# adaptivegenome/openge

Measured on AMD Instinct MI355X. Metric: Mreads/sec sort+dedup (and realign intervals/sec), 1/2/4/8 MI355X, higher is better.
Workload: dtype u8

## Files before the change

openge_amd/csrc/bgzf.hip:

```cpp
#include <hip/hip_runtime.h>

#include <cstdint>
#include <cstdlib>
#include <cstring>
#include <string>
#include <vector>

#include "bam_layout.h"
#include "oge_ctx.h"
#include "records.h"
#include "bgzf_dev.h"

namespace {

using namespace oge_bgzf;
constexpr int kT = 512;
constexpr int kSeg = 64;
constexpr int kSub = kT * kSeg;
constexpr int kNSub = 2;
constexpr int kNSeg = kT * kNSub;
constexpr int kHashBits = 12;
constexpr int kLit = 286, kDist = 30, kCl = 19;
constexpr int kFreq = kLit + kDist;
constexpr int kHdrWords = 144;
// ... 732 lines not shown
    __syncthreads();
    {
        const uint32_t c = lane >= 1 && lane <= M ? hs.cnt[lane] : 0u;
        uint32_t K = c << ((M - lane) & 31);
#pragma unroll
        for (int o = 32; o >= 1; o >>= 1) K += __shfl_xor(K, o, 64);
        if (lane == 0 && K != (1u << M)) {
            const uint32_t one = 1u << M;
            while (K > one) {
                int b = M - 1;
                while (hs.cnt[b] == 0) --b;
                hs.cnt[b]--;
                hs.cnt[b + 1]++;
                K -= 1u << (M - b - 1);
            }
            while (K < one) {
                int b = M;
                while (hs.cnt[b] == 0 || K + (1u << (M - b)) > one) --b;
                hs.cnt[b]--;
                hs.cnt[b - 1]++;
                K += 1u << (M - b);
            }
        }
    }
    __syncthreads();
    {
        uint32_t suf = lane >= 1 && lane <= M ? hs.cnt[lane] : 0u;
#pragma unroll
        for (int o = 1; o < 16; o <<= 1) {
            const uint32_t y = __shfl_down(suf, o, 64);
            if (lane + o < 16) suf += y;
        }
        uint32_t sb[15];
#pragma unroll
        for (int b = 0; b < 15; ++b) sb[b] = (uint32_t)__shfl((int)suf, b + 1, 64);
        for (uint32_t k = lane; k < m; k += 64) {
            uint32_t b = 0;
#pragma unroll
            for (int q = 0; q < 15; ++q) b += (q < M && k < sb[q]) ? 1u : 0u;
            len[hs.sorted[k]] = (uint8_t)b;
        }
    }
    __syncthreads();
    HLCLK(5);
#if OGE_EXP == 3
    if (n == kLit && blockIdx.x == 0 && threadIdx.x == 0)
        printf("huff_lengths lit: keys %llu sort %llu merge %llu depths %llu counts+lengths %llu (m %u)\n",
               (unsigned long long)(g_hl_clk[1] - g_hl_clk[0]), (unsigned long long)(g_hl_clk[2] - g_hl_clk[1]),
               (unsigned long long)(g_hl_clk[3] - g_hl_clk[2]), (unsigned long long)(g_hl_clk[4] - g_hl_clk[3]),
               (unsigned long long)(g_hl_clk[5] - g_hl_clk[4]), m);
#endif
}

__device__ void huff_codes(const uint8_t *len, int n, uint32_t *out) {
    const int lane = threadIdx.x;
    const uint64_t lt = (1ull << lane) - 1;
    uint32_t cnt = 0;
    for (int i0 = 0; i0 < n; i0 += 64) {
        const uint32_t L = i0 + lane < n ? len[i0 + lane] : 0u;
#pragma unroll
        for (int b = 1; b < 16; ++b) {
            const uint32_t c = (uint32_t)__popcll(__ballot(L == (uint32_t)b));
            if (lane == b) cnt += c;
        }
    }
    uint32_t first = 0, code = 0;
#pragma unroll
    for (int b = 1; b < 16; ++b) {
        code = (code + (b > 1 ? (uint32_t)__shfl(cnt, b - 1, 64) : 0u)) << 1;
        if (lane == b) first = code;
    }
    uint32_t run = 0;
    for (int i0 = 0; i0 < n; i0 += 64) {
        const int i = i0 + lane;
        const uint32_t L = i < n ? len[i] : 0u;
        const uint32_t base = (uint32_t)__shfl(run, (int)L, 64) + (uint32_t)__shfl(first, (int)L, 64);
        uint32_t r = 0, add = 0;
#pragma unroll
        for (int b = 1; b < 16; ++b) {
            const uint64_t mk = __ballot(L == (uint32_t)b);
            if (L == (uint32_t)b) r = (uint32_t)__popcll(mk & lt);
            if (lane == b) add = (uint32_t)__popcll(mk);
        }
        run += add;
        if (i < n) out[i] = L ? (__builtin_bitreverse32(base + r) >> (32 - L)) | (L << 16) : 0u;
    }
    __syncthreads();
}

__constant__ uint8_t kClOrder[kCl] = {16, 17, 18, 0, 8, 7, 9, 6, 10, 5, 11, 4, 12, 3, 13, 2, 14, 1, 15};

__device__ __forceinline__ uint32_t len_extra(uint32_t ls) { return ls < 8 ? 0u : ls < 28 ? (ls - 4) >> 2 : 0u; }
__device__ __forceinline__ uint32_t dist_extra(uint32_t ds) { return ds < 4 ? 0u : (ds - 2) >> 1; }

__global__ void __launch_bounds__(64) k_defl_huff(const uint32_t *__restrict__ freq_in, DeflTab *__restrict__ tabs, uint64_t n,
                                                 uint64_t blk0, int level, uint32_t *__restrict__ sizes) {
    __shared__ uint32_t f[kFreq];
    __shared__ uint8_t lens[kFreq];
    __shared__ uint32_t fcl[kCl];
    __shared__ uint8_t lcl[kCl];
    __shared__ uint32_t ccl[kCl];
    __shared__ uint8_t cl_sym[kFreq], cl_ext[kFreq];
    __shared__ uint32_t ncl;
    __shared__ HuffScratch hs;
    const int lane = threadIdx.x;
    DeflTab &T = tabs[blockIdx.x];
#if OGE_EXP == 3
    uint64_t xc[10];
    int xn = 0;
#define XCLK() (xc[xn++] = __builtin_readcyclecounter())
#else
#define XCLK()
#endif
    XCLK();
    uint32_t nzl = 0, nzd = 0;
    for (int i = lane, r = 0; r < (kFreq + 63) / 64; i += 64, ++r) {
        const uint32_t v = i < kFreq ? freq_in[(uint64_t)blockIdx.x * kFreq + i] + (i == 256) : 0u;
        if (i < kFreq) f[i] = v;
        nzl += (uint32_t)__popcll(__ballot(i < kLit && v != 0));
        nzd += (uint32_t)__popcll(__ballot(i >= kLit && i < kFreq && v != 0));
    }
    __syncthreads();
    if (lane == 0 && (nzl < 2 || nzd < 2)) {
        for (int i = 0; nzl < 2 && i < kLit; ++i)
            if (!f[i]) f[i] = 1, ++nzl;
        for (int i = 0; nzd < 2 && i < kDist; ++i)
            if (!f[kLit + i]) f[kLit + i] = 1, ++nzd;
    }
    __syncthreads();
    XCLK();
    huff_lengths(f, kLit, 15, lens, hs);
    XCLK();
    huff_lengths(f + kLit, kDist, 15, lens + kLit, hs);
    XCLK();
    huff_codes(lens, kLit, T.lit);
    huff_codes(lens + kLit, kDist, T.dist);
    XCLK();

    __shared__ uint32_t hlit, hdist;
    __shared__ uint32_t hw[kHdrWords];
    {
        uint32_t la = 0, lb = 0;
        for (int r = 0; r < 5; ++r) {
            const int i = 64 * r + lane;
            const uint64_t mk = __ballot(i < kLit && lens[i] != 0);
            if (mk) la = 64 * r + 64 - __builtin_clzll(mk);
        }
        const uint64_t mkd = __ballot(lane < kDist && lens[kLit + lane] != 0);
        if (mkd) lb = 64 - __builtin_clzll(mkd);
        const uint32_t a = max(la, 257u), b = max(lb, 1u), N = a + b;
        auto val = [&](uint32_t p) -> uint32_t { return p < a ? lens[p] : lens[kLit + p - a]; };
        uint64_t st[5];
#pragma unroll
        for (int r = 0; r < 5; ++r) {
            const uint32_t p = 64 * r + lane;
            st[r] = __ballot(p < N && (p == 0 || p == a || val(p) != val(p - 1)));
        }
        if (lane < kCl) fcl[lane] = 0;
        if (lane == 0) hlit = a, hdist = b;
        __syncthreads();
        uint32_t base = 0;
#pragma unroll
        for (int r = 0; r < 5; ++r) {
            const uint32_t p = 64 * r + lane;
            const bool start = (st[r] >> lane) & 1;
            uint32_t R = 0, v = 0, ntok = 0;
            if (start) {
                uint32_t nx = N;
                const uint64_t rest = lane < 63 ? st[r] & (~0ull << (lane + 1)) : 0ull;
                if (rest) {
                    nx = 64 * r + __builtin_ctzll(rest);
                } else {
#pragma unroll
                    for (int r2 = 4; r2 > r; --r2)
                        if (st[r2]) nx = 64 * r2 + __builtin_ctzll(st[r2]);
                }
                R = min(nx, N) - p;
                v = val(p);
                if (v == 0) {
                    const uint32_t rm = R % 138;
                    ntok = R / 138 + (rm >= 3 ? 1 : rm);
                } else {
                    const uint32_t rm = (R - 1) % 6;
                    ntok = 1 + (R - 1) / 6 + (rm >= 3 ? 1 : rm);
                }
            }
            uint32_t inc = ntok;
#pragma unroll
            for (int o = 1; o < 64; o <<= 1) {
                const uint32_t y = __shfl_up(inc, o, 64);
                if (lane >= (uint32_t)o) inc += y;
            }
            uint32_t k = base + inc - ntok;
            base += __shfl(inc, 63, 64);
            if (start) {
                auto tok = [&](uint32_t sym, uint32_t ext) {
                    cl_sym[k] = (uint8_t)sym;
                    cl_ext[k] = (uint8_t)ext;
                    atomicAdd(&fcl[sym], 1u);
                    ++k;
                };
                if (v == 0) {
                    for (uint32_t q = 0; q < R / 138; ++q) tok(18, 127);
                    const uint32_t rm = R % 138;
                    if (rm >= 11) tok(18, rm - 11);
                    else if (rm >= 3) tok(17, rm - 3);
                    else
                        for (uint32_t q = 0; q < rm; ++q) tok(0, 0);
                } else {
                    tok(v, 0);
                    for (uint32_t q = 0; q < (R - 1) / 6; ++q) tok(16, 3);
                    const uint32_t rm = (R - 1) % 6;
                    if (rm >= 3) tok(16, rm - 3);
                    else
                        for (uint32_t q = 0; q < rm; ++q) tok(v, 0);
                }
            }
        }
        __syncthreads();
        if (lane == 0) {
            ncl = base;
            uint32_t nz = 0;
            for (int i = 0; i < kCl; ++i) nz += fcl[i] != 0;
            for (int i = 0; nz < 2 && i < kCl; ++i)
                if (!fcl[i]) fcl[i] = 1, ++nz;
        }
    }
    __syncthreads();
    XCLK();
    huff_lengths(fcl, kCl, 7, lcl, hs);
    huff_codes(lcl, kCl, ccl);
    XCLK();
    {
        for (int i = lane; i < kHdrWords; i += 64) hw[i] = 0;
        const uint64_t mh = __ballot(lane >= 4 && lane < kCl && lcl[kClOrder[lane]] != 0);
        const uint32_t hclen = mh ? 64 - __builtin_clzll(mh) : 4u;
        __syncthreads();
        auto orbits = [&](uint32_t at, uint32_t v, uint32_t nb) {
            if (!nb) return;
            const uint32_t w = at >> 5, sh = at & 31;
            atomicOr(&hw[w], v << sh);
            if (sh + nb > 32) atomicOr(&hw[w + 1], v >> (32 - sh));
        };
        if (lane == 0) orbits(0, 1u | (2u << 1) | ((hlit - 257) << 3) | ((hdist - 1) << 8) | ((hclen - 4) << 13), 17);
        if ((uint32_t)lane < hclen) orbits(17 + 3 * lane, lcl[kClOrder[lane]], 3);
        const uint32_t n = ncl;
        uint32_t at = 17 + 3 * hclen;
        for (uint32_t t0 = 0; t0 < n; t0 += 64) {
            const uint32_t t = t0 + lane;
            uint32_t nb = 0, v = 0;
            if (t < n) {
                const uint32_t sym = cl_sym[t], c = ccl[sym], cb = c >> 16;
                const uint32_t eb = sym == 16 ? 2u : sym == 17 ? 3u : sym == 18 ? 7u : 0u;
                nb = cb + eb;
                v = (c & 0xffff) | ((uint32_t)cl_ext[t] << cb);
            }
            uint32_t inc = nb;
#pragma unroll
            for (int o = 1; o < 64; o <<= 1) {
                const uint32_t y = __shfl_up(inc, o, 64);
                if (lane >= (uint32_t)o) inc += y;
            }
            orbits(at + inc - nb, v, nb);
            at += __shfl(inc, 63, 64);
        }
        __syncthreads();
        for (uint32_t i = lane; i < (at + 31) / 32; i += 64) T.hdr[i] = hw[i];
        if (lane == 0) {
            T.hdr_bits = at;
            ncl = at;
        }
    }
    __syncthreads();
    uint32_t bits = 0;
    for (int i = lane; i < kFreq; i += 64) {
        const uint32_t fr = freq_in[(uint64_t)blockIdx.x * kFreq + i] + (i == 256);
        const uint32_t ex = i < 257 ? 0u : i < kLit ? len_extra(i - 257) : dist_extra(i - kLit);
        bits += fr * (lens[i] + ex);
    }
#pragma unroll
    for (int o = 32; o >= 1; o >>= 1) bits += __shfl_xor(bits, o, 64);
    if (lane == 0) {
        const uint64_t start = (blk0 + blockIdx.x) * kPay;
        const uint32_t len = (uint32_t)min<uint64_t>(kPay, n - start);
        const uint32_t dbytes = (ncl + bits + 7) / 8;
        const uint32_t stored = level == 0 || dbytes > len + 5;
        const uint32_t total = stored ? 18 + 5 + len + 8 : 18 + dbytes + 8;
        T.stored = stored;
        T.total = total;
        sizes[blockIdx.x] = total;
    }
#if OGE_EXP == 3
    XCLK();
    if (lane == 0 && blockIdx.x < 4 && blk0 == 0)
        printf("huff-exp blk %u: load %llu lit-lengths %llu dist-lengths %llu codes %llu rle %llu cl %llu header+size %llu\n",
               blockIdx.x, (unsigned long long)(xc[1] - xc[0]), (unsigned long long)(xc[2] - xc[1]), (unsigned long long)(xc[3] - xc[2]),
               (unsigned long long)(xc[4] - xc[3]), (unsigned long long)(xc[5] - xc[4]), (unsigned long long)(xc[6] - xc[5]),
               (unsigned long long)(xc[7] - xc[6]));
#endif
}

struct LdsBits {
    uint32_t *base;
    uint64_t acc;
    uint32_t nacc, wpos;
    __device__ __forceinline__ void init(uint32_t *b, uint32_t bit) { base = b, acc = 0, nacc = bit & 31, wpos = bit >> 5; }
    __device__ __forceinline__ void put(uint32_t v, uint32_t nb) {
        acc |= (uint64_t)v << nacc;
        nacc += nb;
        if (nacc >= 32) {
            const uint32_t w = (uint32_t)acc;
            atomicOr(base + wpos, w);
            ++wpos;
            acc >>= 32;
            nacc -= 32;
        }
    }
    __device__ __forceinline__ void finish() {
        if (nacc && (uint32_t)acc) atomicOr(base + wpos, (uint32_t)acc);
    }
};

__device__ __forceinline__ uint32_t ct_entry(uint32_t i, const uint32_t *tlit) {
    if (i < 256) {
        const uint32_t c = tlit[i];
        return (c & 0xffff) | (c >> 16) << 24;
    }
    uint32_t sym, nb, ev;
    len_code(i - 256 + 3, sym, nb, ev);
    const uint32_t c = tlit[sym];
    return ((c & 0xffff) | (ev << (c >> 16))) | ((c >> 16) + nb) << 24;
}
__device__ __forceinline__ void dist_bits(uint32_t D, const uint32_t *dist, uint32_t &v, uint32_t &n) {
    const uint32_t d = D - 1, lg = 31 - __builtin_clz(d | 1);
    const bool small = d < 4;
    const uint32_t dnb = small ? 0u : lg - 1;
    const uint32_t dsym = small ? d : 2 * lg + ((d >> ((lg - 1) & 31)) & 1);
    const uint32_t dev = d & ((1u << dnb) - 1);
    const uint32_t c = dist[dsym];
    v = (c & 0xffff) | (dev << (c >> 16));
    n = (c >> 16) + dnb;
}
__device__ __forceinline__ uint32_t match_bits(uint32_t m, const uint32_t *ct, const uint32_t *dist) {
    uint32_t dv, dn;
    dist_bits((m & 0x7fff) + 1, dist, dv, dn);
    return (ct[256 + ((m >> 15) & 255)] >> 24) + dn;
}

__device__ __forceinline__ void seg_load(const uint8_t *s, uint32_t s0, uint32_t len, uint32_t (&w)[16]) {
    if (s0 + kSeg <= len && !((uintptr_t)(s + s0) & 15)) {
        const uint4 *g = (const uint4 *)(s + s0);
#pragma unroll
        for (int k = 0; k < 4; ++k) {
            const uint4 v = g[k];
            w[4 * k] = v.x, w[4 * k + 1] = v.y, w[4 * k + 2] = v.z, w[4 * k + 3] = v.w;
        }
    } else {
#pragma unroll
        for (int k = 0; k < 16; ++k) {
            uint32_t v = 0;
#pragma unroll
            for (int b = 0; b < 4; ++b)
                if (s0 + 4 * k + b < len) v |= (uint32_t)s[s0 + 4 * k + b] << (8 * b);
            w[k] = v;
        }
    }
}

#ifndef OGE_EMIT_MPRE
#define OGE_EMIT_MPRE 8
#endif
constexpr int kMPre = OGE_EMIT_MPRE;
__device__ __forceinline__ void seg_tokens(const uint32_t *mp, uint32_t nm, uint32_t (&m)[kMPre]) {
    const uint32_t last = nm ? nm - 1 : 0;
#pragma unroll
    for (int k = 0; k < kMPre; ++k) m[k] = mp[(uint64_t)min((uint32_t)k, last) * kNSeg];
}

__device__ __forceinline__ uint32_t seg_bits(const uint32_t (&w)[16], uint64_t lm, uint32_t nm, const uint32_t *mp,
                                             const uint32_t (&m)[kMPre], const uint32_t *ct, const uint32_t *dist) {
    uint32_t bits = 0;
#pragma unroll
    for (int g = 0; g < 4; ++g) {
        uint32_t c[16];
#pragma unroll
        for (int i = 0; i < 16; ++i) c[i] = ct[(w[4 * g + (i >> 2)] >> (8 * (i & 3))) & 0xff];
#pragma unroll
        for (int i = 0; i < 16; ++i) bits += (lm >> (16 * g + i)) & 1 ? c[i] >> 24 : 0u;
    }
#pragma unroll
    for (int k = 0; k < kMPre; ++k)
        if ((uint32_t)k < nm) bits += match_bits(m[k], ct, dist);
    for (uint32_t k = kMPre; k < nm; ++k) bits += match_bits(mp[(uint64_t)k * kNSeg], ct, dist);
    return bits;
}

__device__ __forceinline__ void seg_emit(const uint32_t (&w)[16], uint64_t lm, uint32_t nm, const uint32_t *mp,
                                         uint32_t (&m)[kMPre], const uint32_t *ct, const uint32_t *dist, uint32_t *img,
                                         uint32_t bit) {
    uint32_t k = 0, cur = m[0], moff = nm ? (cur >> 23) : 64u;
    uint32_t lc, dv, dn;
    auto look = [&](uint32_t tok) {
        lc = ct[256 + ((tok >> 15) & 255)];
        dist_bits((tok & 0x7fff) + 1, dist, dv, dn);
    };
    look(cur);
    LdsBits bw;
    bw.init(img, bit);
#pragma unroll
    for (int g = 0; g < 4; ++g) {
        uint32_t c[16];
#pragma unroll
        for (int i = 0; i < 16; ++i) c[i] = ct[(w[4 * g + (i >> 2)] >> (8 * (i & 3))) & 0xff];
#pragma unroll
        for (int i0 = 0; i0 < 16; i0 += 2) {
            const int i = 16 * g + i0;
            const uint32_t a = (lm >> i) & 1 ? c[i0] : 0u, b = (lm >> (i + 1)) & 1 ? c[i0 + 1] : 0u;
            bw.put((a & 0xffffff) | ((b & 0xffffff) << (a >> 24)), (a >> 24) + (b >> 24));
            if (((uint32_t)i | 1u) == (moff | 1u)) {
#if OGE_EXP == 8
                ++k;
#pragma unroll
                for (int q = 0; q + 1 < kMPre; ++q) m[q] = m[q + 1];
                moff = k < nm && k < (uint32_t)kMPre ? m[0] >> 23 : 64u;
#else
                bw.put(lc & 0xffffff, lc >> 24);
                bw.put(dv, dn);
                ++k;
#pragma unroll
                for (int q = 0; q + 1 < kMPre; ++q) m[q] = m[q + 1];
                if (k < nm) {
                    cur = k < (uint32_t)kMPre ? m[0] : mp[(uint64_t)k * kNSeg];
                    moff = cur >> 23;
                    look(cur);
                } else {
                    moff = 64;
                }
#endif
            }
        }
    }
    bw.finish();
}

struct EmitCrc {
    uint32_t crctab[4][256];
    uint32_t zp[17][32];
    uint32_t zl[32][16];
    uint32_t crcs[kT / 64];
};
constexpr uint32_t kLdsGranule = 1280;
constexpr uint32_t kLdsCu = 163840;
constexpr uint32_t kEmitFixed = (512 + kDist + kNSeg + kT / 64 + 2) * 4;
constexpr uint32_t emit_lds(uint32_t cap) { return (cap + 16 + kEmitFixed + kLdsGranule - 1) / kLdsGranule * kLdsGranule; }
#ifndef OGE_EMIT_SMALL_CAP
#define OGE_EMIT_SMALL_CAP (46 * 1024)
#endif
constexpr uint32_t kEmitSmallCap = OGE_EMIT_SMALL_CAP;
static_assert(kEmitSmallCap % 1024 == 0 && 3 * emit_lds(kEmitSmallCap) <= kLdsCu && 3 * emit_lds(kEmitSmallCap + 1024) > kLdsCu,
              "small emit instance: three workgroups per CU, and no larger cap does");
static_assert(sizeof(EmitCrc) <= kEmitSmallCap, "the CRC tables alias the image");

template <uint32_t CAP>
__device__ __forceinline__ void emit_block(const uint32_t bi, const uint8_t *__restrict__ src, uint64_t n, uint64_t blk0,
                                           const uint64_t *__restrict__ lmask, const uint8_t *__restrict__ nmatch,
                                           const uint32_t *__restrict__ mlist, const DeflTab *__restrict__ tabs,
                                           const uint32_t *__restrict__ zpow, const uint32_t *__restrict__ offs,
                                           const uint64_t *__restrict__ cbase, uint8_t *__restrict__ dst) {
    constexpr bool kSmall = CAP < kSlot;
    const DeflTab &T = tabs[bi];
    const uint32_t total = T.total, stored = T.stored, hb = T.hdr_bits;
    __shared__ __align__(16) uint32_t img[CAP / 4 + 4];
    __shared__ uint32_t ct[512], dist[kDist];
    __shared__ uint32_t scan[kNSeg];
    __shared__ uint32_t wsum[kT / 64];
    __shared__ __align__(16) uint32_t crc_own[kSmall ? 1 : sizeof(EmitCrc) / 4];
    __shared__ uint32_t sh_crc;
    EmitCrc &C = *(EmitCrc *)(kSmall ? img : crc_own);
    int tid = threadIdx.x;
    asm volatile("" : "+v"(tid));
    const int t = tid, lane = t & 63, wv = t >> 6;
    const uint64_t blk = blk0 + bi;
    const uint64_t start = blk * kPay;
    const uint32_t len = (uint32_t)min<uint64_t>(kPay, n - start);
    const uint8_t *s = src + start;
    for (int i = t; i < 512; i += kT) ct[i] = ct_entry(i, T.lit);
    for (int i = t; i < kDist; i += kT) dist[i] = T.dist[i];
    crc_setup<kT>(C.crctab, C.zp, zpow, t);
    for (int i = t; i < 32 * 16; i += kT) C.zl[i >> 4][i & 15] = zpow[17 * 32 + i];
    if (!kSmall)
        for (uint32_t i = t; i < (total + 15) / 16; i += kT) ((uint4 *)img)[i] = make_uint4(0, 0, 0, 0);
    __syncthreads();
    {
        const uint32_t c = crc_global512x4l(s, len, C.crctab, C.zl, C.zp, C.crcs, t);
        if (t == 0) sh_crc = c;
    }
    if (kSmall) {
        __syncthreads();
        for (uint32_t i = t; i < (total + 15) / 16; i += kT) ((uint4 *)img)[i] = make_uint4(0, 0, 0, 0);
        if (stored) __syncthreads();
    }
    const uint32_t bsize = total - 1;
    if (stored) {
        for (uint32_t i = t; i < len; i += kT) ((uint8_t *)img)[23 + i] = s[i];
    } else {
        const uint32_t s0a = t * kSeg, s0b = kSub + t * kSeg;
        const uint64_t sga = (uint64_t)bi * kNSeg + t, sgb = sga + kT;
        const uint64_t lma = s0a < len ? lmask[sga] : 0, lmb = s0b < len ? lmask[sgb] : 0;
        const uint32_t nma = s0a < len ? nmatch[sga] : 0, nmb = s0b < len ? nmatch[sgb] : 0;
        const uint32_t *mpa = mlist + ((uint64_t)bi * kMaxM) * kNSeg + t, *mpb = mpa + kT;
        uint32_t ca, cb;
        {
            uint32_t w[16], m[kMPre];
            seg_load(s, s0a, len, w);
            seg_tokens(mpa, nma, m);
            ca = seg_bits(w, lma, nma, mpa, m, ct, dist);
            seg_load(s, s0b, len, w);
            seg_tokens(mpb, nmb, m);
            cb = seg_bits(w, lmb, nmb, mpb, m, ct, dist);
        }
        scan[t] = ca;
        scan[kT + t] = cb;
        __syncthreads();
        {
            const uint32_t a = scan[2 * t], b = scan[2 * t + 1];
            uint32_t x = a + b, inc = x;
#pragma unroll
            for (int o = 1; o < 64; o <<= 1) {
                const uint32_t y = __shfl_up(inc, o);
                if (lane >= o) inc += y;
            }
            if (lane == 63) wsum[wv] = inc;
            __syncthreads();
            uint32_t pre = 0;
            for (int q = 0; q < wv; ++q) pre += wsum[q];
            const uint32_t ex = pre + inc - x;
            __syncthreads();
            scan[2 * t] = ex;
            scan[2 * t + 1] = ex + a;
        }
        __syncthreads();
        for (uint32_t i = t; i < (hb + 31) / 32; i += kT) {
            const uint32_t v = T.hdr[i];
            atomicOr(img + 4 + i, v << 16);
            if (v >> 16) atomicOr(img + 5 + i, v >> 16);
        }
        {
            uint32_t w[16], m[kMPre];
            if (ca) {
                seg_load(s, s0a, len, w);
                seg_tokens(mpa, nma, m);
                seg_emit(w, lma, nma, mpa, m, ct, dist, img, 144 + hb + scan[t]);
            }
            if (cb) {
                uint32_t tb = t;
                asm volatile("" : "+v"(tb));
                const uint64_t lm2 = lmask[(uint64_t)bi * kNSeg + kT + tb];
                seg_load(s, s0b, len, w);
                seg_tokens(mpb, nmb, m);
                seg_emit(w, lm2, nmb, mpb, m, ct, dist, img, 144 + hb + scan[kT + t]);
            }
        }
        if (t == kT - 1) {
            const uint32_t body_end = 144 + hb + scan[kNSeg - 1] + cb;
            LdsBits bw;
            bw.init(img, body_end);
            const uint32_t c = T.lit[256];
            bw.put(c & 0xffff, c >> 16);
            bw.finish();
        }
    }
    __syncthreads();
    uint8_t *ib = (uint8_t *)img;
    if (t == 0) {
        img[0] = 0x04088b1fu;
        img[1] = 0;
        img[2] = 0x0006ff00u;
        img[3] = 0x00024342u;
        ib[16] = (uint8_t)bsize, ib[17] = (uint8_t)(bsize >> 8);
        if (stored) {
            ib[18] = 1;
            ib[19] = (uint8_t)len, ib[20] = (uint8_t)(len >> 8);
            ib[21] = (uint8_t)~len, ib[22] = (uint8_t)(~len >> 8);
        }
        const uint32_t q = total - 8;
        for (int b = 0; b < 4; ++b) ib[q + b] = (uint8_t)(sh_crc >> (8 * b)), ib[q + 4 + b] = (uint8_t)(len >> (8 * b));
    }
    __syncthreads();
    uint8_t *D = dst + *cbase + offs[bi];
    const uint32_t sh = (uint32_t)((uintptr_t)D & 3);
    OGE_G uint32_t *A = (OGE_G uint32_t *)((uintptr_t)D & ~(uintptr_t)3);
    const uint32_t nwords = (total + sh + 3) / 4;
    for (uint32_t g = t; g < nwords; g += kT) {
        const int32_t r0 = (int32_t)(4 * g) - (int32_t)sh;
        if (r0 >= 0 && r0 + 4 <= (int32_t)total) {
            A[g] = ld32(img, (uint32_t)r0);
        } else {
            for (int i = 0; i < 4; ++i) {
                const int32_t r = r0 + i;
                if (r >= 0 && r < (int32_t)total) ((OGE_G uint8_t *)(A + g))[i] = ib[r];
            }
        }
    }
}

template <uint32_t CAP>
__global__ void __launch_bounds__(kT, CAP < kSlot ? 6 : 4) k_defl_emit(const uint8_t *__restrict__ src, uint64_t n, uint64_t blk0,
                                                     const uint64_t *__restrict__ lmask, const uint8_t *__restrict__ nmatch,
                                                     const uint32_t *__restrict__ mlist, const DeflTab *__restrict__ tabs,
                                                     const uint32_t *__restrict__ zpow, const uint32_t *__restrict__ offs,
                                                     const uint64_t *__restrict__ cbase, uint8_t *__restrict__ dst, uint32_t cap,
                                                     const uint32_t *__restrict__ big) {
    if (CAP < kSlot) {
        if (tabs[blockIdx.x].total <= cap) emit_block<CAP>(blockIdx.x, src, n, blk0, lmask, nmatch, mlist, tabs, zpow, offs, cbase, dst);
    } else {
        const uint32_t nq = big ? big[0] : blockIdx.x + 1;
#pragma unroll 1
        for (uint32_t q = blockIdx.x; q < nq; q += gridDim.x) {
            const uint32_t bi = big ? big[4 + q] : q;
            if (!big && tabs[bi].total <= cap) break;
            emit_block<CAP>(bi, src, n, blk0, lmask, nmatch, mlist, tabs, zpow, offs, cbase, dst);
            __syncthreads();
        }
    }
}

constexpr uint32_t kMaxChunk = 16384, kPer = kMaxChunk / 1024;
__global__ void __launch_bounds__(1024) k_scan_chunk(const uint32_t *__restrict__ in, uint32_t n, uint32_t *__restrict__ out,
                                                     uint32_t cap, unsigned long long *__restrict__ nsmall,
                                                     uint32_t *__restrict__ big) {
    __shared__ uint32_t ws[16], wb[16];
    const uint32_t t = threadIdx.x, lane = t & 63, w = t >> 6;
    uint32_t a[kPer], v = 0, nbig = 0, small = 0;
#pragma unroll
    for (uint32_t i = 0; i < kPer; ++i) {
        a[i] = kPer * t + i < n ? in[kPer * t + i] : 0;
        v += a[i];
        small += a[i] && a[i] <= cap;
        nbig += a[i] > cap;
    }
#pragma unroll
    for (int d = 32; d >= 1; d >>= 1) small += __shfl_xor(small, d, 64);
    if (lane == 0 && small) atomicAdd(nsmall, (unsigned long long)small);
    uint32_t x = v, xb = nbig;
#pragma unroll
    for (int d = 1; d < 64; d <<= 1) {
        const uint32_t y = __shfl_up(x, d, 64), yb = __shfl_up(xb, d, 64);
        if (lane >= (uint32_t)d) x += y, xb += yb;
    }
    if (lane == 63) ws[w] = x, wb[w] = xb;
    __syncthreads();
    if (t < 16) {
        uint32_t s = ws[t], z = s, sb = wb[t], zb = sb;
        for (int d = 1; d < 16; d <<= 1) {
            const uint32_t y = __shfl_up(z, d, 16), yb = __shfl_up(zb, d, 16);
            if ((t & 15) >= (uint32_t)d) z += y, zb += yb;
        }
        ws[t] = z - s;
        wb[t] = zb - sb;
        if (t == 15) big[0] = zb;
    }
    __syncthreads();
    uint32_t excl = ws[w] + x - v, rank = wb[w] + xb - nbig;
#pragma unroll
    for (uint32_t i = 0; i < kPer; ++i) {
        if (kPer * t + i < n) out[kPer * t + i] = excl;
        excl += a[i];
        if (a[i] > cap) big[4 + rank++] = kPer * t + i;
    }
}

__global__ void k_defl_advance(uint64_t *base, uint64_t *cbase, const uint32_t *offs, const uint32_t *sizes, uint32_t nb) {
    if (threadIdx.x == 0 && blockIdx.x == 0) {
        const uint64_t b = *base;
        *cbase = b;
        *base = b + (uint64_t)offs[nb - 1] + sizes[nb - 1];
    }
}

__global__ void k_fix_bins(uint8_t *__restrict__ recs, const uint64_t *__restrict__ off, uint64_t n) {
    const uint64_t i = (uint64_t)blockIdx.x * blockDim.x + threadIdx.x;
    if (i >= n) return;
    uint8_t *r = recs + off[i];
    oge_wr_u16(r + OGE_OFF_BIN, oge_rec_bin(r));
}

}


extern "C" uint64_t oge_bgzf_bound(uint64_t n) { return ((n + kPay - 1) / kPay) * (uint64_t)kSlot; }

extern "C" uint32_t oge_defl_emit_cap(void) { return kEmitSmallCap; }

static uint32_t emit_cap_now() {
    const char *e = getenv("OGE_DEFL_EMIT_CAP");
    if (!e || !*e) return kEmitSmallCap;
    return (uint32_t)std::min<unsigned long long>(strtoull(e, nullptr, 10), kEmitSmallCap);
}

extern "C" int oge_bgzf_deflate_dev(oge_ctx *ctx, const uint8_t *d_src, uint64_t n, int level, uint8_t *d_dst,
                                    uint64_t dst_cap, uint64_t *out_bytes) {
    if (!ctx) return oge_fail(nullptr, OGE_ERR_ARG, "null ctx");
    if (!out_bytes || (n && (!d_src || !d_dst))) return oge_fail(ctx, OGE_ERR_ARG, "null buffer");
    if (level < 0 || level > 9) return oge_fail(ctx, OGE_ERR_ARG, "level must be 0..9");
    const int depth = level >= 9 ? 32 : level == 8 ? 8 : 1, lazy = level >= 8 ? 1 : 0;
    const int search = level == 0 ? OGE_DEFL_FAST : ctx->deflate_search;
    if (dst_cap < oge_bgzf_bound(n)) return oge_fail(ctx, OGE_ERR_ARG, "dst_cap < oge_bgzf_bound(n)");
    OgeCall call(ctx, false);
    *out_bytes = 0;
    if (!n) return OGE_OK;
    const uint64_t nblk = (n + kPay - 1) / kPay;
    const int ncu = ctx->cu_count();
#ifndef OGE_DEFL_STREAMS
#define OGE_DEFL_STREAMS 3
#endif
#ifndef OGE_DEFL_CHUNK
#define OGE_DEFL_CHUNK kMaxChunk
#endif
    static_assert(OGE_DEFL_CHUNK <= kMaxChunk, "k_scan_chunk bound");
    constexpr uint64_t kPerPay = (uint64_t)kNSeg * 8 + kNSeg + (uint64_t)kMaxM * kNSeg * 4 + kFreq * 4 + sizeof(DeflTab) + 8;
    const int S0 = nblk > 4096 ? OGE_DEFL_STREAMS : 1;
    uint64_t chunk = std::min<uint64_t>(nblk, OGE_DEFL_CHUNK);
    if (chunk > 4096) {
        size_t fr = 0, tot = 0;
        if (hipMemGetInfo(&fr, &tot) != hipSuccess) fr = 0;
        uint64_t held = 0;
        for (int s = 0; s < 3; ++s) {
            const auto it = ctx->bufs.find("defl_mlist" + std::to_string(s));
            if (it != ctx->bufs.end()) held += it->second.cap / ((uint64_t)kMaxM * kNSeg * 4) * kPerPay;
        }
        while (chunk > 4096 && (uint64_t)S0 * chunk * kPerPay > (fr + held) / 4) chunk = std::max<uint64_t>(4096, chunk / 2);
    }
    static_assert(OGE_DEFL_STREAMS >= 1 && OGE_DEFL_STREAMS <= 3, "deflate: 1-3 streams");
    const int S = nblk > chunk ? OGE_DEFL_STREAMS : 1;
    struct Bufs {
        uint64_t *lmask, *cbase;
        uint32_t *mlist, *freq, *sizes, *offs, *big;
        uint8_t *nmatch;
        DeflTab *tabs;
        hipStream_t st;
    } B[3];
    for (int s = 0; s < S; ++s) {
        const std::string x = std::to_string(s);
        B[s].lmask = (uint64_t *)ctx->ws(("defl_lmask" + x).c_str(), chunk * kNSeg * 8);
        B[s].nmatch = (uint8_t *)ctx->ws(("defl_nmatch" + x).c_str(), chunk * kNSeg);
        B[s].mlist = (uint32_t *)ctx->ws(("defl_mlist" + x).c_str(), chunk * kMaxM * kNSeg * 4);
        B[s].freq = (uint32_t *)ctx->ws(("defl_freq" + x).c_str(), chunk * kFreq * 4);
        B[s].tabs = (DeflTab *)ctx->ws(("defl_tabs" + x).c_str(), chunk * sizeof(DeflTab));
        B[s].sizes = (uint32_t *)ctx->ws(("defl_sizes" + x).c_str(), chunk * 4 + 16);
        B[s].offs = (uint32_t *)ctx->ws(("defl_offs" + x).c_str(), chunk * 4 + 16);
        B[s].cbase = (uint64_t *)ctx->ws(("defl_cbase" + x).c_str(), 16);
        B[s].big = (uint32_t *)ctx->ws(("defl_big" + x).c_str(), chunk * 4 + 16);
        B[s].st = S == 1 ? ctx->stream : ctx->side_stream(s);
        if (!B[s].lmask || !B[s].nmatch || !B[s].mlist || !B[s].freq || !B[s].tabs || !B[s].sizes || !B[s].offs ||
            !B[s].cbase || !B[s].big || !B[s].st)
            return OGE_ERR_HIP;
    }
    uint32_t *zpow = (uint32_t *)ctx->ws("defl_zpow", (17 * 32 + 32 * 16) * 4);
    uint64_t *base = (uint64_t *)ctx->ws("defl_base", 16);
    if (!zpow || !base) return OGE_ERR_HIP;
    static struct {
        uint32_t z[17][32], zl[32][16];
    } zh = [] {
        decltype(zh) v;
        crc_zpow(v.z);
        crc_zlane<16>(v.z, 128, &v.zl[0][0]);
        return v;
    }();
    OGE_HIP_TRY(ctx, hipMemcpyAsync(zpow, &zh, sizeof(zh), hipMemcpyHostToDevice, ctx->stream));
    OGE_HIP_TRY(ctx, hipMemsetAsync(base, 0, 16, ctx->stream));
    const uint32_t ecap = emit_cap_now();
    OgeStage stage(ctx, "bgzf_deflate");
    hipEvent_t ev[4];
    for (auto &e : ev) OGE_HIP_TRY(ctx, hipEventCreateWithFlags(&e, hipEventDisableTiming));
    struct Evs {
        hipEvent_t *e;
        ~Evs() {
            for (int i = 0; i < 4; ++i) hipEventDestroy(e[i]);
        }
    } evs{ev};
    OGE_HIP_TRY(ctx, hipEventRecord(ev[3], ctx->stream));
    for (int s = 0; s < S; ++s)
        if (B[s].st != ctx->stream) OGE_HIP_TRY(ctx, hipStreamWaitEvent(B[s].st, ev[3], 0));
    uint64_t k = 0;
    for (uint64_t b0 = 0; b0 < nblk; b0 += chunk, ++k) {
        const uint32_t nb = (uint32_t)std::min(chunk, nblk - b0);
        Bufs &u = B[k % S];
        const uint32_t pg = (uint32_t)std::min<uint64_t>(nb, (uint64_t)ncu);
#define OGE_PARSE_X(C, N, S) \
    k_defl_parse_x<C, N, S><<<pg, kTP, 0, u.st>>>(d_src, n, b0, nb, u.lmask, u.nmatch, u.mlist, u.freq, depth, lazy)
        if (search == OGE_DEFL_FAST && depth > 1)
            k_defl_parse<true><<<pg, kTP, 0, u.st>>>(d_src, n, b0, nb, u.lmask, u.nmatch, u.mlist, u.freq, depth, lazy);
        else if (search == OGE_DEFL_FAST)
            k_defl_parse<false><<<pg, kTP, 0, u.st>>>(d_src, n, b0, nb, u.lmask, u.nmatch, u.mlist, u.freq, 1, 0);
        else if (search == OGE_DEFL_NEAR)
            depth > 1 ? OGE_PARSE_X(true, true, false) : OGE_PARSE_X(false, true, false);
        else if (search == OGE_DEFL_SPAN)
            depth > 1 ? OGE_PARSE_X(true, false, true) : OGE_PARSE_X(false, false, true);
        else
            depth > 1 ? OGE_PARSE_X(true, true, true) : OGE_PARSE_X(false, true, true);
#undef OGE_PARSE_X
        OGE_LAUNCH_CHECK(ctx);
        k_defl_huff<<<nb, 64, 0, u.st>>>(u.freq, u.tabs, n, b0, level, u.sizes);
        OGE_LAUNCH_CHECK(ctx);
        k_scan_chunk<<<1, 1024, 0, u.st>>>(u.sizes, nb, u.offs, ecap, (unsigned long long *)(base + 1), u.big);
        OGE_LAUNCH_CHECK(ctx);
        if (k) OGE_HIP_TRY(ctx, hipStreamWaitEvent(u.st, ev[(k - 1) % S], 0));
        k_defl_advance<<<1, 64, 0, u.st>>>(base, u.cbase, u.offs, u.sizes, nb);
        OGE_LAUNCH_CHECK(ctx);
        OGE_HIP_TRY(ctx, hipEventRecord(ev[k % S], u.st));
        if (ecap) {
            k_defl_emit<kEmitSmallCap><<<nb, kT, 0, u.st>>>(d_src, n, b0, u.lmask, u.nmatch, u.mlist, u.tabs, zpow, u.offs, u.cbase,
                                                            d_dst, ecap, nullptr);
            OGE_LAUNCH_CHECK(ctx);
            k_defl_emit<kSlot><<<std::min<uint32_t>(nb, 2 * (uint32_t)ncu), kT, 0, u.st>>>(d_src, n, b0, u.lmask, u.nmatch, u.mlist, u.tabs,
                                                                                           zpow, u.offs, u.cbase, d_dst, ecap, u.big);
        } else {
            k_defl_emit<kSlot><<<nb, kT, 0, u.st>>>(d_src, n, b0, u.lmask, u.nmatch, u.mlist, u.tabs, zpow, u.offs, u.cbase, d_dst, 0, nullptr);
        }
        OGE_LAUNCH_CHECK(ctx);
    }
    if (S > 1) {
        for (int s = 0; s < S; ++s) {
            OGE_HIP_TRY(ctx, hipEventRecord(ev[s], B[s].st));
            OGE_HIP_TRY(ctx, hipStreamWaitEvent(ctx->stream, ev[s], 0));
        }
    }
    stage.end();
    uint64_t total[2] = {0, 0};
    OGE_HIP_TRY(ctx, hipMemcpyAsync(total, base, 16, hipMemcpyDeviceToHost, ctx->stream));
    OGE_HIP_TRY(ctx, hipStreamSynchronize(ctx->stream));
    *out_bytes = total[0];
    ctx->counters["defl_emit_small"] += total[1];
    ctx->counters["defl_emit_big"] += nblk - total[1];
    static const bool tr = getenv("OGE_TRACE_DEFL") != nullptr;
    if (tr)
        fprintf(stderr, "[oge defl] %llu blocks, %llu bytes, emit cap %u: %llu small, %llu big\n", (unsigned long long)nblk,
                (unsigned long long)total[0], ecap, (unsigned long long)total[1], (unsigned long long)(nblk - total[1]));
    return OGE_OK;
}

extern "C" int oge_bgzf_deflate(oge_ctx *ctx, const uint8_t *src, uint64_t n, int level, uint8_t *dst, uint64_t dst_cap,
                                uint64_t *out_bytes) {
    if (!ctx) return oge_fail(nullptr, OGE_ERR_ARG, "null ctx");
    if (!out_bytes || (n && (!src || !dst))) return oge_fail(ctx, OGE_ERR_ARG, "null buffer");
    hipSetDevice(ctx->device);
    *out_bytes = 0;
    if (!n) return OGE_OK;
    const uint64_t bound = oge_bgzf_bound(n);
    uint8_t *ds = (uint8_t *)ctx->ws("defl_hsrc", n + 16);
    uint8_t *dd = (uint8_t *)ctx->ws("defl_hdst", bound);
    if (!ds || !dd) return OGE_ERR_HIP;
    OGE_HIP_TRY(ctx, hipMemcpyAsync(ds, src, n, hipMemcpyHostToDevice, ctx->stream));
    uint64_t got = 0;
    int rc = oge_bgzf_deflate_dev(ctx, ds, n, level, dd, bound, &got);
    if (rc) return rc;
    if (got > dst_cap) return oge_fail(ctx, OGE_ERR_ARG, "dst_cap too small for the compressed stream");
    OGE_HIP_TRY(ctx, hipMemcpyAsync(dst, dd, got, hipMemcpyDeviceToHost, ctx->stream));
    OGE_HIP_TRY(ctx, hipStreamSynchronize(ctx->stream));
    *out_bytes = got;
    return OGE_OK;
}

// ... 10 lines not shown
```

Measured before the change: 328.0.

## Defer match emission in deflate emit to a second pass with recorded bit offsets

The emit loop no longer carries preloaded match tokens or looks up length and distance codes inline. It reserves bit gaps for matches using per-match bit counts packed by seg_bits into a SegMatches bitset, records their offsets in packed 10-bit registers, and writes the match codes in a separate loop afterwards with direct atomicOr. The bit accumulator also shrinks from 64-bit to 32-bit. The aim is to cut register pressure and branch divergence in the unrolled literal loop. The cost is extra atomics and a second pass over matches, plus recomputing literal offsets for matches beyond nine.

New measurement: 329.0, median of 3. Within noise of the previous version (+0.3%).

```diff
diff --git a/openge_amd/csrc/bgzf.hip b/openge_amd/csrc/bgzf.hip
--- a/openge_amd/csrc/bgzf.hip
+++ b/openge_amd/csrc/bgzf.hip
@@ -1058,22 +1058,30 @@
 
 struct LdsBits {
     uint32_t *base;
-    uint64_t acc;
-    uint32_t nacc, wpos;
+    uint32_t acc, nacc, wpos;
     __device__ __forceinline__ void init(uint32_t *b, uint32_t bit) { base = b, acc = 0, nacc = bit & 31, wpos = bit >> 5; }
     __device__ __forceinline__ void put(uint32_t v, uint32_t nb) {
-        acc |= (uint64_t)v << nacc;
+        const uint32_t sh = nacc;
+        acc |= v << sh;
         nacc += nb;
         if (nacc >= 32) {
-            const uint32_t w = (uint32_t)acc;
-            atomicOr(base + wpos, w);
+            atomicOr(base + wpos, acc);
             ++wpos;
-            acc >>= 32;
+            acc = (v >> 1) >> (31 - sh);
             nacc -= 32;
         }
     }
+    __device__ __forceinline__ uint32_t skip(uint32_t nb) {
+        atomicOr(base + wpos, acc);
+        const uint32_t at = (wpos << 5) | nacc;
+        acc = 0;
+        nacc += nb;
+        wpos += nacc >> 5;
+        nacc &= 31;
+        return at;
+    }
     __device__ __forceinline__ void finish() {
-        if (nacc && (uint32_t)acc) atomicOr(base + wpos, (uint32_t)acc);
+        if (nacc && acc) atomicOr(base + wpos, acc);
     }
 };
 
@@ -1133,8 +1141,14 @@
     for (int k = 0; k < kMPre; ++k) m[k] = mp[(uint64_t)min((uint32_t)k, last) * kNSeg];
 }
 
+struct SegMatches {
+    uint64_t start, lo, hi;
+};
+static_assert(6 * kMaxM <= 128 && 6 * kMPre <= 64, "the matches' bit counts fit lo:hi, the preloaded ones lo");
+
 __device__ __forceinline__ uint32_t seg_bits(const uint32_t (&w)[16], uint64_t lm, uint32_t nm, const uint32_t *mp,
-                                             const uint32_t (&m)[kMPre], const uint32_t *ct, const uint32_t *dist) {
+                                             const uint32_t (&m)[kMPre], const uint32_t *ct, const uint32_t *dist,
+                                             SegMatches &sm) {
     uint32_t bits = 0;
 #pragma unroll
     for (int g = 0; g < 4; ++g) {
@@ -1144,25 +1158,36 @@
 #pragma unroll
         for (int i = 0; i < 16; ++i) bits += (lm >> (16 * g + i)) & 1 ? c[i] >> 24 : 0u;
     }
+    sm.start = 0, sm.lo = 0, sm.hi = 0;
 #pragma unroll
     for (int k = 0; k < kMPre; ++k)
-        if ((uint32_t)k < nm) bits += match_bits(m[k], ct, dist);
-    for (uint32_t k = kMPre; k < nm; ++k) bits += match_bits(mp[(uint64_t)k * kNSeg], ct, dist);
+        if ((uint32_t)k < nm) {
+            const uint32_t b = match_bits(m[k], ct, dist);
+            bits += b;
+            sm.start |= 1ull << (m[k] >> 23);
+            sm.lo |= (uint64_t)b << (6 * k);
+        }
+    for (uint32_t k = kMPre; k < nm; ++k) {
+        const uint32_t tok = mp[(uint64_t)k * kNSeg], b = match_bits(tok, ct, dist), o = 6 * k;
+        bits += b;
+        sm.start |= 1ull << (tok >> 23);
+        if (o < 64) {
+            sm.lo |= (uint64_t)b << o;
+            sm.hi |= (uint64_t)b >> (64 - o);
+        } else {
+            sm.hi |= (uint64_t)b << (o - 64);
+        }
+    }
     return bits;
 }
 
+constexpr uint32_t kNoted = 9;
 __device__ __forceinline__ void seg_emit(const uint32_t (&w)[16], uint64_t lm, uint32_t nm, const uint32_t *mp,
-                                         uint32_t (&m)[kMPre], const uint32_t *ct, const uint32_t *dist, uint32_t *img,
-                                         uint32_t bit) {
-    uint32_t k = 0, cur = m[0], moff = nm ? (cur >> 23) : 64u;
-    uint32_t lc, dv, dn;
-    auto look = [&](uint32_t tok) {
-        lc = ct[256 + ((tok >> 15) & 255)];
-        dist_bits((tok & 0x7fff) + 1, dist, dv, dn);
-    };
-    look(cur);
+                                         SegMatches sm, const uint8_t *sp, const uint32_t *ct, const uint32_t *dist,
+                                         uint32_t *img, uint32_t bit) {
     LdsBits bw;
     bw.init(img, bit);
+    uint32_t n0 = 0, n1 = 0, n2 = 0;
 #pragma unroll
     for (int g = 0; g < 4; ++g) {
         uint32_t c[16];
@@ -1173,30 +1198,58 @@
             const int i = 16 * g + i0;
             const uint32_t a = (lm >> i) & 1 ? c[i0] : 0u, b = (lm >> (i + 1)) & 1 ? c[i0 + 1] : 0u;
             bw.put((a & 0xffffff) | ((b & 0xffffff) << (a >> 24)), (a >> 24) + (b >> 24));
-            if (((uint32_t)i | 1u) == (moff | 1u)) {
-#if OGE_EXP == 8
-                ++k;
-#pragma unroll
-                for (int q = 0; q + 1 < kMPre; ++q) m[q] = m[q + 1];
-                moff = k < nm && k < (uint32_t)kMPre ? m[0] >> 23 : 64u;
-#else
-                bw.put(lc & 0xffffff, lc >> 24);
-                bw.put(dv, dn);
-                ++k;
-#pragma unroll
-                for (int q = 0; q + 1 < kMPre; ++q) m[q] = m[q + 1];
-                if (k < nm) {
-                    cur = k < (uint32_t)kMPre ? m[0] : mp[(uint64_t)k * kNSeg];
-                    moff = cur >> 23;
-                    look(cur);
-                } else {
-                    moff = 64;
-                }
+            if ((uint32_t)(sm.start >> i) & 3u) {
+                const uint32_t rel = bw.skip((uint32_t)sm.lo & 63u) - bit;
+                n0 = __builtin_amdgcn_alignbit(n1, n0, 10);
+                n1 = __builtin_amdgcn_alignbit(n2, n1, 10);
+                n2 = (n2 >> 10) | (rel << 22);
+                sm.lo = (sm.lo >> 6) | (sm.hi << 58);
+                sm.hi >>= 6;
+            }
+        }
+    }
+    bw.finish();
+#if OGE_EXP != 8
+    if (nm) {
+        const uint32_t over = nm > kNoted ? nm - kNoted : 0u, sh = 96u - 10u * (nm - over);
+        if (sh >= 64) {
+            n0 = n2, n1 = 0, n2 = 0;
+        } else if (sh >= 32) {
+            n0 = n1, n1 = n2, n2 = 0;
+        }
+        n0 = __builtin_amdgcn_alignbit(n1, n0, sh & 31);
+        n1 = __builtin_amdgcn_alignbit(n2, n1, sh & 31);
+        n2 >>= sh & 31;
+        uint32_t x = 0, lb = 0, mb = 0;
+        uint32_t nxt = mp[0];
+        for (uint32_t k = 0; k < nm; ++k) {
+            const uint32_t tok = nxt;
+            nxt = mp[(uint64_t)min(k + 1, nm - 1) * kNSeg];
+            const uint32_t lc = ct[256 + ((tok >> 15) & 255)], ln = lc >> 24;
+            uint32_t dv, dn;
+            dist_bits((tok & 0x7fff) + 1, dist, dv, dn);
+            uint32_t rel;
+            if (k < over) {
+                for (const uint32_t q = tok >> 23; x < q; ++x)
+                    if ((lm >> x) & 1) lb += ct[sp[x]] >> 24;
+                rel = lb + mb;
+            } else {
+                rel = n0 & 1023u;
+                n0 = __builtin_amdgcn_alignbit(n1, n0, 10);
+                n1 = __builtin_amdgcn_alignbit(n2, n1, 10);
+                n2 >>= 10;
+            }
+            mb += ln + dn;
+            const uint32_t pos = bit + rel, s = pos & 31;
+            uint32_t *wp = img + (pos >> 5);
+            const uint64_t v = (uint64_t)(lc & 0xffffff) | ((uint64_t)dv << ln), lo = v << s;
+            const uint32_t w1 = (uint32_t)(lo >> 32), w2 = (uint32_t)((v >> 33) >> (31 - s));
+            atomicOr(wp, (uint32_t)lo);
+            if (w1) atomicOr(wp + 1, w1);
+            if (w2) atomicOr(wp + 2, w2);
+        }
+    }
 #endif
-            }
-        }
-    }
-    bw.finish();
 }
 
 struct EmitCrc {
@@ -1266,14 +1319,15 @@
         const uint32_t nma = s0a < len ? nmatch[sga] : 0, nmb = s0b < len ? nmatch[sgb] : 0;
         const uint32_t *mpa = mlist + ((uint64_t)bi * kMaxM) * kNSeg + t, *mpb = mpa + kT;
         uint32_t ca, cb;
+        SegMatches sma, smb;
         {
             uint32_t w[16], m[kMPre];
             seg_load(s, s0a, len, w);
             seg_tokens(mpa, nma, m);
-            ca = seg_bits(w, lma, nma, mpa, m, ct, dist);
+            ca = seg_bits(w, lma, nma, mpa, m, ct, dist, sma);
             seg_load(s, s0b, len, w);
             seg_tokens(mpb, nmb, m);
-            cb = seg_bits(w, lmb, nmb, mpb, m, ct, dist);
+            cb = seg_bits(w, lmb, nmb, mpb, m, ct, dist, smb);
         }
         scan[t] = ca;
         scan[kT + t] = cb;
@@ -1302,19 +1356,17 @@
             if (v >> 16) atomicOr(img + 5 + i, v >> 16);
         }
         {
-            uint32_t w[16], m[kMPre];
+            uint32_t w[16];
             if (ca) {
                 seg_load(s, s0a, len, w);
-                seg_tokens(mpa, nma, m);
-                seg_emit(w, lma, nma, mpa, m, ct, dist, img, 144 + hb + scan[t]);
+                seg_emit(w, lma, nma, mpa, sma, s + s0a, ct, dist, img, 144 + hb + scan[t]);
             }
             if (cb) {
                 uint32_t tb = t;
                 asm volatile("" : "+v"(tb));
                 const uint64_t lm2 = lmask[(uint64_t)bi * kNSeg + kT + tb];
                 seg_load(s, s0b, len, w);
-                seg_tokens(mpb, nmb, m);
-                seg_emit(w, lm2, nmb, mpb, m, ct, dist, img, 144 + hb + scan[kT + t]);
+                seg_emit(w, lm2, nmb, mpb, smb, s + s0b, ct, dist, img, 144 + hb + scan[kT + t]);
             }
         }
         if (t == kT - 1) {
```
